# cmcqueen/lzs-compression

Measured on AMD Instinct MI355X. Metric: input GB/s on 64KiB blocks, bit-exact vs C ref, higher is better.
Workload: dtype u8

## Files before the change

lzs_compression_amd/csrc/kernels/compress_wg.inc:

```

#ifdef LZS_WGV_WG_WAVES
constexpr uint32_t kW = LZS_WGV_WG_WAVES;
#else
constexpr uint32_t kW = 4;
#endif
static_assert(kW == 4 || kW == 8, "four or eight waves per workgroup");
constexpr uint32_t kWgThreads  = 64u * kW;
constexpr uint32_t kChunkStride = 64u * kW;
constexpr uint32_t kWgRing      = kW == 8 ? 8192u : 4096u;
constexpr uint32_t kWgRingMask  = kWgRing - 1u, kWgRingWords = kWgRing / 4u;
constexpr uint32_t kRefillUnit  = 128u * kW;
#ifndef LZS_WG_HEAD3
#define LZS_WG_HEAD3 1792
#endif
#ifndef LZS_WG_HEAD2
#define LZS_WG_HEAD2 1024
#endif
#ifdef LZS_WGV_HEAD3
constexpr uint32_t kWgHead3    = LZS_WGV_HEAD3;
#else
constexpr uint32_t kWgHead3    = LZS_WG_HEAD3;
#endif
#ifdef LZS_WGV_HEAD2
constexpr uint32_t kWgHead2    = LZS_WGV_HEAD2;
#else
constexpr uint32_t kWgHead2    = LZS_WG_HEAD2;
#endif
#ifdef LZS_WGV_NO3
constexpr bool kNo3 = true;
#else
constexpr bool kNo3 = false;
#endif
#ifdef LZS_WGV_EXIT8
constexpr bool kExit8 = true;
typedef uint8_t exit_t;
#else
constexpr bool kExit8 = false;
typedef uint16_t exit_t;
#endif
#ifdef LZS_WGV_CHAIN_SAFE
constexpr bool kChainSafe = true;
#else
constexpr bool kChainSafe = false;
#endif
constexpr uint32_t kWgHead2Shift = kWgHead2 == 4096 ? 4 : kWgHead2 == 2048 ? 5 : kWgHead2 == 1024 ? 6 : kWgHead2 == 512 ? 7 : 8;
#ifdef LZS_WGV_POOL
constexpr uint32_t kWgPool     = LZS_WGV_POOL;
#else
constexpr uint32_t kWgPool     = 128u * kW;
#endif
static_assert(kWgPool == 128u * kW || (kW == 4 && kWgPool == 256), "a wave parses one or two chunks of 64 positions");
constexpr int      kCh         = (int)(kWgPool / kChunkStride);
constexpr uint32_t kWgLinkN    = (2047u + 2u * kWgPool + 63u) / 64u * 64u;
constexpr uint32_t kWgResN     = 2 * kWgPool;
constexpr uint32_t kWgBitWords = 64u * kW;
constexpr uint32_t kBitMask    = 32u * kWgBitWords - 1u;
constexpr uint32_t kOpen       = 0xFFFFu;
constexpr uint32_t kExtOpen    = 63;
#ifndef LZS_SUBSTEPS
#define LZS_SUBSTEPS 2
#endif
#ifdef LZS_WGV_SUBSTEPS
constexpr int kSubsteps = LZS_WGV_SUBSTEPS;
#else
constexpr int kSubsteps = LZS_SUBSTEPS;
#endif
#ifndef LZS_HOPS
#define LZS_HOPS 2
#endif
#ifdef LZS_WGV_HOPS
#define LZS_HOPS_HERE LZS_WGV_HOPS
#else
#define LZS_HOPS_HERE LZS_HOPS
#endif
constexpr int kHops = LZS_HOPS_HERE;
#ifdef LZS_WGV_HOP_END
constexpr bool kHopEnd = true;
#else
constexpr bool kHopEnd = false;
#endif
#ifdef LZS_WGV_HOPS_LAST
constexpr int kHopsLast = LZS_WGV_HOPS_LAST;
#else
constexpr int kHopsLast = kHops;
#endif
constexpr uint32_t kExtMax     = 59;
constexpr uint32_t kOpenStep   = 4080;
#ifndef LZS_RUN_ROUNDS
#define LZS_RUN_ROUNDS 2
#endif
#ifndef LZS_RUN_POOL
#define LZS_RUN_POOL 128
#endif
constexpr uint32_t kRunRounds  = LZS_RUN_ROUNDS;
constexpr uint32_t kRunPool    = LZS_RUN_POOL;

struct __attribute__((aligned(16))) BlkLds {
    uint32_t ring[kWgRingWords + 4];
    uint32_t head3[kNo3 ? 1 : kWgHead3];
    uint32_t head2[kWgHead2];
    uint16_t link3[kNo3 ? 2 : kWgLinkN];
    uint16_t link2[kWgLinkN];
    uint16_t res[kWgResN];
    exit_t   exitfn[kExit8 && kWgPool < 2u * kWgThreads ? 2u * kWgThreads : kWgPool];
    uint32_t bits[kWgBitWords];
    uint32_t chunk_bits[2 * kW];
    uint32_t nextp;
    uint32_t bcast[8];
#ifdef LZS_PAD_LDS
    uint32_t pad[LZS_PAD_LDS / 4];
#endif
};

#ifndef LZS_HASH3_MUL
#define LZS_HASH3_MUL 0x1EB419u
#endif
#ifndef LZS_HASH2_MUL
#define LZS_HASH2_MUL 0xCFC8AE9Bu
#endif
#ifdef LZS_WGV_HASH3_MUL
constexpr uint32_t kHash3Mul = LZS_WGV_HASH3_MUL;
#else
constexpr uint32_t kHash3Mul = LZS_HASH3_MUL;
#endif
#ifdef LZS_WGV_HASH2_MUL
constexpr uint32_t kHash2Mul = LZS_WGV_HASH2_MUL;
#else
constexpr uint32_t kHash2Mul = LZS_HASH2_MUL;
#endif
__device__ __forceinline__ uint32_t wg_hash3x4(uint32_t t) { return __umulhi(__umul24(t, kHash3Mul), 4u * kWgHead3) & ~3u; }

__device__ __forceinline__ uint32_t wg_slot_base(uint32_t B) { return ((B >> 6) % (kWgLinkN / 64u)) * 64u; }
__device__ __forceinline__ uint32_t wg_link_slot(uint32_t at)
{
    if constexpr ((kWgLinkN & (kWgLinkN - 1u)) == 0u) return at & (kWgLinkN - 1u);
    uint32_t b, r;
#ifdef LZS_WGV_LEAN
    asm("v_add_u16 %0, %2, %1" : "=v"(b) : "v"(at), "n"(kWgLinkN));
#else
    asm("v_add_u16 %0, %1, %2" : "=v"(b) : "v"(at), "v"(kWgLinkN));
#endif
    asm("v_min_u16 %0, %1, %2" : "=v"(r) : "v"(at), "v"(b));
    return r;
}

__device__ __forceinline__ uint32_t lcp12(uint32_t x0, uint32_t x1, uint32_t x2)
{
    uint32_t f0, f1, f2;
    asm("v_ffbl_b32 %0, %1" : "=v"(f0) : "v"(x0));
    asm("v_ffbl_b32 %0, %1" : "=v"(f1) : "v"(x1));
    asm("v_ffbl_b32 %0, %1" : "=v"(f2) : "v"(x2));
    const uint32_t a = f1 | 32u, b = f2 | 64u;
    const uint32_t m = f0 < a ? (f0 < b ? f0 : b) : (a < b ? a : b);
    return m >> 3;
}

__device__ __forceinline__ void bits_or(uint32_t *ring, uint32_t words, uint32_t at, uint32_t value, uint32_t width)
{
    const uint32_t sh = at & 31u, d = (at >> 5) & (words - 1);
    const uint64_t v = (uint64_t)value << (64u - sh - width);
    const uint32_t hi = (uint32_t)(v >> 32), lo = (uint32_t)v;
    __hip_atomic_fetch_or(&ring[d], hi, __ATOMIC_RELAXED, __HIP_MEMORY_SCOPE_WORKGROUP);
    if (lo) __hip_atomic_fetch_or(&ring[(d + 1) & (words - 1)], lo, __ATOMIC_RELAXED, __HIP_MEMORY_SCOPE_WORKGROUP);
}

struct WgOut {
    uint32_t flushed;
    uint32_t head;
    uint8_t *dst;
    uint32_t cap;
    bool     aligned4;
    uint32_t limit;
    bool     ored;
};

__device__ __forceinline__ uint32_t wg_bit_at(const WgOut &o) { return ((o.flushed << 3) + o.head) & kBitMask; }

__device__ __forceinline__ void wg_store_quarter(const WgOut &o, BlkLds &L, uint32_t lane)
{
    const uint32_t slot = ((o.flushed >> 8) & (kWgBitWords / 64u - 1u)) * 64u + lane;
    const uint32_t v = __builtin_bswap32(L.bits[slot]);
    L.bits[slot] = 0;
    const uint32_t at = o.flushed + 4 * lane;
    if (o.ored) {
        if (v) atomicOr(reinterpret_cast<unsigned int *>(o.dst + at), v);
        return;
    }
    if (o.aligned4 && at + 4 <= o.limit) {
        *reinterpret_cast<uint32_t *>(o.dst + at) = v;
    } else {
        for (uint32_t k = 0; k < 4; k++)
            if (at + k < o.limit) o.dst[at + k] = (uint8_t)(v >> (8 * k));
    }
}

__device__ __forceinline__ uint16_t *wg_dummy(BlkLds &L) { return reinterpret_cast<uint16_t *>(L.exitfn) + threadIdx.x; }

__device__ __forceinline__ uint32_t wg_ring_byte(const uint32_t *ring, uint32_t q) { return reinterpret_cast<const uint8_t *>(ring)[q & kWgRingMask]; }
__device__ __forceinline__ void wg_read12(const uint32_t *ring, uint32_t q, uint32_t &w0, uint32_t &w1, uint32_t &w2)
{
    const uint32_t a = (q & kWgRingMask) >> 2;
    const uint32_t d0 = ring[a], d1 = ring[a + 1], d2 = ring[a + 2], d3 = ring[a + 3];
    w0 = __builtin_amdgcn_alignbyte(d1, d0, q);
    w1 = __builtin_amdgcn_alignbyte(d2, d1, q);
    w2 = __builtin_amdgcn_alignbyte(d3, d2, q);
}

typedef __attribute__((address_space(3))) uint32_t lds_u32_t;
typedef __attribute__((address_space(3))) uint16_t lds_u16_t;
__device__ __forceinline__ uint32_t lds_off(const void *p) { return (uint32_t)(uintptr_t)(__attribute__((address_space(3))) const void *)p; }
__device__ __forceinline__ lds_u32_t *lds_word(uint32_t off) { return (lds_u32_t *)(uintptr_t)off; }
__device__ __forceinline__ lds_u16_t *lds_half(uint32_t off) { return (lds_u16_t *)(uintptr_t)off; }

__device__ __forceinline__ void wg_hash_range(BlkLds &L, uint32_t B0, uint32_t Be, uint32_t lane, uint32_t wave)
{
    const uint32_t head3_at = lds_off(L.head3), head2_at = lds_off(L.head2);
    const uint32_t dummy3 = lds_off(L.exitfn) + 4u * lane, dummy2 = dummy3 + 256u;
    for (uint32_t B = B0 + 64u * wave; B < Be; B += kChunkStride * kCh) {
        uint32_t e[kCh][5];
#pragma unroll
        for (int j = 0; j < kCh; j++) {
            const uint32_t p = B + kChunkStride * j + lane;
            const uint32_t a = ((p - 4u) & kWgRingMask) >> 2;
#pragma unroll
            for (int k = 0; k < 5; k++) e[j][k] = L.ring[a + k];
        }
#pragma unroll
        for (int j = 0; j < kCh; j++) {
            const uint32_t Bj = B + kChunkStride * j, p = Bj + lane;
            const uint32_t tcur = __builtin_amdgcn_alignbyte(e[j][2], e[j][1], p);
            const uint32_t rot = __builtin_amdgcn_alignbit(e[j][0], e[j][0], 8);
            const uint32_t x = (e[j][0] ^ rot) | (e[j][1] ^ e[j][0]) | (e[j][2] ^ e[j][0]) | (e[j][3] ^ e[j][0]) | (e[j][4] ^ e[j][0]);
            const bool skip = x == 0u;
            const uint32_t g2 = head2_at + (((tcur * kHash2Mul) >> (kWgHead2Shift - 2u)) & (4u * (kWgHead2 - 1)));
            const uint32_t a2 = skip ? dummy2 : g2;
            const uint32_t sl = wg_slot_base(Bj) + lane;
            uint16_t *const dummy16 = wg_dummy(L);
            if constexpr (!kNo3) {
                const uint32_t g3 = opaque(head3_at + wg_hash3x4(tcur));
                const uint32_t a3 = skip ? dummy3 : g3;
                *(Bj < Be ? &L.link3[sl] : dummy16) = (uint16_t)a3;
            }
            *(Bj < Be ? &L.link2[sl] : dummy16) = (uint16_t)a2;
        }
    }
}

template <int K>
__device__ __forceinline__ void wg_chain_group(BlkLds &L, uint32_t B, uint32_t &slot, uint32_t lane, uint32_t half, uint16_t *links)
{
    (void)half;
    uint32_t at[K], old[K];
    uint16_t *la[K];
#pragma unroll
    for (int j = 0; j < K; j++) {
        la[j] = &links[slot + lane];
        at[j] = *la[j];
        slot = slot + 64u >= kWgLinkN ? slot + 64u - kWgLinkN : slot + 64u;
    }
#pragma unroll
    for (int j = 0; j < K; j++) {
        const uint32_t p = B + 64u * j + lane;
        old[j] = __hip_atomic_exchange(lds_word(at[j]), p, __ATOMIC_RELAXED, __HIP_MEMORY_SCOPE_WORKGROUP);
    }
#pragma unroll
    for (int j = 0; j < K; j++) {
        const uint32_t p = B + 64u * j + lane;
        const uint32_t d = p - old[j] < kNoLink ? p - old[j] : kNoLink;
        *la[j] = (uint16_t)d;
    }
}

__device__ __forceinline__ void wg_chain_batch_safe(BlkLds &L, uint32_t B, uint32_t &slot, uint32_t lane, uint32_t half, uint16_t *links)
{
    (void)half;
    const uint32_t at = links[slot + lane];
    const uint32_t p = B + lane;
    const bool ins = at - lds_off(L.exitfn) >= (uint32_t)sizeof(L.exitfn);
    uint64_t same = __builtin_amdgcn_ballot_w64(ins);
#pragma unroll
    for (uint32_t bit = 2; bit < 15u; bit++) {
        const bool set = (at >> bit) & 1u;
        const uint64_t bb = __builtin_amdgcn_ballot_w64(set);
        same &= set ? bb : ~bb;
    }
    const uint64_t lower = same & ((1ull << lane) - 1ull);
    const bool top = (same >> lane >> 1) == 0ull;
    const uint32_t old = ins ? *lds_word(at) : ~0u;
    __builtin_amdgcn_wave_barrier();
    uint32_t d = kNoLink;
    if (ins) {
        if (lower) d = lane - (63u - (uint32_t)__builtin_clzll(lower));
        else       d = p - old < kNoLink ? p - old : kNoLink;
        if (top) *lds_word(at) = p;
    }
    links[slot + lane] = (uint16_t)d;
    slot = slot + 64u >= kWgLinkN ? slot + 64u - kWgLinkN : slot + 64u;
    __builtin_amdgcn_wave_barrier();
}

__device__ __forceinline__ void wg_chain_range(BlkLds &L, uint32_t B0, uint32_t Be, uint32_t lane, uint32_t wave)
{
    if (wave >= 2u) return;
    if (kNo3 && wave == 0u) return;
    const bool two = wave == 1u;
    uint16_t *const links = two ? L.link2 : L.link3;
    const uint32_t half = two ? 2u : 0u;
    uint32_t slot = wg_slot_base(B0);
    uint32_t B = B0;
    if constexpr (kChainSafe) {
        for (; B < Be; B += 64u) wg_chain_batch_safe(L, B, slot, lane, half, links);
        return;
    }
#ifdef LZS_WGV_PRIO
    __builtin_amdgcn_s_setprio(3);
#endif
    for (; B + 256u <= Be; B += 256u) wg_chain_group<4>(L, B, slot, lane, half, links);
    for (; B < Be; B += 64u) wg_chain_group<1>(L, B, slot, lane, half, links);
#ifdef LZS_WGV_PRIO
    __builtin_amdgcn_s_setprio(2);
#endif
}

#ifdef LZS_PROFILE
#ifdef LZS_PROFILE_COUNTS
#define SEARCH_PROF_PARAMS , uint32_t *prof_acc
#else
#define SEARCH_PROF_PARAMS , unsigned long long *prof_acc
#endif
#define SEARCH_PROF_ARGS , prof_acc
#else
#define SEARCH_PROF_PARAMS
#define SEARCH_PROF_ARGS
#endif
__device__ __forceinline__ void wg_extend(BlkLds &L, uint32_t Pb, uint32_t entry, uint32_t npos, uint32_t n, uint32_t lane, uint32_t wave,
                                          uint32_t (&rr)[2] SEARCH_PROF_PARAMS)
{
    PROF_ITER_DECL;
    constexpr uint32_t kRoom = kTokenMax + kExtMax + 1;
#pragma unroll
    for (int h = 0; h < kCh; h++) {
        const uint32_t gi = kChunkStride * h + 64u * wave + lane;
        rr[h] = 0;
        if (64u * wave + kChunkStride * h >= npos) continue;
        const uint32_t p = Pb + gi;
        const uint32_t k = L.res[p & (kWgResN - 1)];
        const uint32_t off = (0u - k) & 0xFFFu;
        const uint32_t len = off ? (k + 0xFFFu) >> 12 : 0u;
        const uint32_t r = off | (len << 11);
        const bool need = gi >= entry && gi < npos && len == kSearchCap && n - p > kSearchCap;
#ifdef LZS_ABLATE_EXTEND
        const uint64_t needs = 0ull;
#else
        const uint64_t needs = __builtin_amdgcn_ballot_w64(need);
#endif
        if (needs == 0ull) {
            rr[h] = r | ((len > kTokenMax ? len - kTokenMax : 0u) << 15);
            continue;
        }
        PROF_COUNT(19, 1);
        const uint32_t left = (uint32_t)__builtin_amdgcn_ds_bpermute((int)((lane - 1u) << 2), (int)r);
        const bool head = need && !(lane > 0u && ((needs >> (lane - 1u)) & 1ull) != 0ull && ((left ^ r) & 0x7FFFu) == 0u);
        const uint64_t heads_all = __builtin_amdgcn_ballot_w64(head);
        const uint64_t ends = (heads_all | ~needs) >> lane >> 1;
        const uint32_t runlen = ends ? (uint32_t)__builtin_ctzll(ends) : 63u - lane;
        uint32_t total = kSearchCap;
        if (head) {
            const uint32_t room = n - p < kRoom ? n - p : kRoom;
            total = kSearchCap + runlen < room ? kSearchCap + runlen : room;
            while (total < room) {
                PROF_ITER;
                uint32_t a0, a1, a2, b0, b1, b2;
                wg_read12(L.ring, p + total, a0, a1, a2);
                wg_read12(L.ring, p + total - off, b0, b1, b2);
                uint32_t e = lcp12(a0 ^ b0, a1 ^ b1, a2 ^ b2);
                e = e < 12u ? e : 12u;
                e = e < room - total ? e : room - total;
                total += e;
                if (e < 12u) break;
            }
        }
        PROF_ITER_DONE(27);
        const uint64_t heads = heads_all & ((2ull << lane) - 1ull);
        const uint32_t hp = heads ? 63u - (uint32_t)__builtin_clzll(heads) : lane;
        const uint32_t th = (uint32_t)__builtin_amdgcn_ds_bpermute((int)(hp << 2), (int)total);
        uint32_t ext = len >= kTokenMax ? len - kTokenMax : 0u;
        if (need) ext = th >= kRoom ? kExtOpen : th - (lane - hp) - kTokenMax;
        rr[h] = r | (ext << 15);
    }
}

struct Walk {
    uint32_t p, t0, t1, t2;
    uint32_t nreach, myslot;
    uint32_t nback;
    int32_t key;
    uint32_t cap;
    uint32_t nfirst2;
    const uint16_t *links;
    uint16_t *resp;
    uint32_t pb, probe;
};
constexpr int32_t kKeyNone3 = 0x2000, kKeyNone2 = 0x1000;

template <bool HE>
__device__ __forceinline__ void wg_search(BlkLds &L, Walk &W, uint32_t Pb, uint32_t pend, uint32_t n, uint32_t lane, bool lit, bool drain SEARCH_PROF_PARAMS)
{
    const uint32_t slot0 = wg_slot_base(Pb);
    uint16_t *const dummy = wg_dummy(L);
    PROF_ITER_DECL;
    bool pool_done = false;
    uint32_t p = W.p, t0 = W.t0, t1 = W.t1, t2 = W.t2, nreach = W.nreach, myslot = W.myslot;
    uint32_t nback = W.nback, cap = W.cap, nfirst2 = W.nfirst2;
    uint32_t pb = W.pb, probe = W.probe;
    int32_t key = W.key;
    const uint16_t *links = W.links;
    uint16_t *resp = W.resp;
#ifdef LZS_WGV_LEAN
    const uint32_t vFFF = 0xFFFu, vRC = kWgRingMask & ~3u, vRM = kWgRingMask;
#else
    const uint32_t vFFF = opaque(0xFFFu), vRC = opaque(kWgRingMask & ~3u);
    const uint32_t vRM = kWgRingMask == 0xFFFu ? vFFF : opaque(kWgRingMask);
#endif
    const uint8_t *const ring8 = reinterpret_cast<const uint8_t *>(L.ring);
    (void)vFFF; (void)vRM;
    for (;;) {
        const uint64_t idle = __builtin_amdgcn_ballot_w64(nback == 0u);
        const uint32_t nidle = (uint32_t)__builtin_popcountll(idle);
        if (!pool_done && nidle >= kRefillMin) {
            uint32_t basep = 0;
            if (lane == 0) asm volatile("ds_add_rtn_u32 %0, %1, %2\n\ts_waitcnt lgkmcnt(0)" : "=v"(basep) : "v"(lds_off(&L.nextp)), "v"(nidle) : "memory");
            basep = uniform(basep);
            pool_done = basep + nidle >= pend;
            const uint32_t rank = __builtin_amdgcn_mbcnt_hi((uint32_t)(idle >> 32),
                                  __builtin_amdgcn_mbcnt_lo((uint32_t)idle, 0u));
            const uint32_t np = basep + rank;
            const bool take = nback == 0u && np < pend;
            PROF_COUNT(9, 1);
            PROF_COUNT(10, __builtin_popcountll(__builtin_amdgcn_ballot_w64(take)));
            PROF_COUNT(43, __builtin_amdgcn_ballot_w64(take) == 0ull);
            PROF_T0;
            if (take) {
                *resp = (uint16_t)key;
                p = np;
                wg_read12(L.ring, p, t0, t1, t2);
                const uint32_t before = wg_ring_byte(L.ring, p - 1u);
                uint32_t sl = slot0 + (p - Pb);
                sl = sl >= kWgLinkN ? sl - kWgLinkN : sl;
                myslot = sl;
                const uint32_t l3 = kNo3 ? kNoLink : (uint32_t)L.link3[sl], l2 = L.link2[sl];
                const uint32_t lim = n - p < kSearchCap ? n - p : kSearchCap;
                const bool maybe1 = p >= 1u && ((t0 ^ ((t0 << 8) | before)) & 0xFFFFu) == 0;
                uint32_t len1 = 0;
                if (__builtin_amdgcn_ballot_w64(maybe1) != 0ull) {
                    PROF_ITER;
                    len1 = lcp12(t0 ^ ((t0 << 8) | before), t1 ^ ((t1 << 8) | (t0 >> 24)), t2 ^ ((t2 << 8) | (t1 >> 24)));
                    len1 = len1 < lim ? len1 : lim;
                }
                const bool seeded = maybe1 && len1 >= 2u;
                const bool capped = seeded && len1 == lim;
                const uint32_t reach = p < kWindow ? p : kWindow;
                nreach = ~reach;
#ifdef LZS_ABLATE_STEPS
                const bool walk3 = false, walk2 = false;
#else
                const bool walk3 = !kNo3 && lim >= 3u && !capped && l3 <= reach && (seeded || !lit);
                const bool walk2 = lim >= 2u && !capped && (kNo3 || !seeded) && l2 <= reach;
#endif
                nfirst2 = 0u - (walk2 ? l2 : kNoLink);
                nback = walk3 ? 0u - l3 : (walk2 ? nfirst2 : 0u);
                key = seeded ? (int32_t)((len1 << 12) - 1u) : (walk3 ? kKeyNone3 : kKeyNone2);
                cap = (walk3 || lit || kNo3) ? lim : 2u;
                links = walk3 ? L.link3 : L.link2;
                uint16_t *const slot = &L.res[p & (kWgResN - 1)];
                resp = slot;
                cap = (walk3 || walk2) ? cap : 0u;
#if LZS_HOPS_HERE
                pb = p + (((uint32_t)key + 0xFFFu) >> 12);
                probe = wg_ring_byte(L.ring, pb);
#endif
            }
            PROF_T1(14);
            PROF_ITER_DONE(18);
        }
        if (pool_done && __builtin_amdgcn_ballot_w64(nback != 0u && (drain || p < Pb)) == 0ull) break;
        PROF_COUNT(11, 1);
        PROF_COUNT(8 + 4, __builtin_popcountll(__builtin_amdgcn_ballot_w64(nback != 0u)));
        PROF_T0B;
#pragma unroll
        for (int sub = 0; sub < kSubsteps; sub++) {
#if LZS_HOPS_HERE
            const int nhops = (HE && sub == kSubsteps - 1) ? kHopsLast : kHops;
#pragma unroll
            for (int hop = 0; hop < nhops; hop++) {
                const uint32_t cb = ring8[(pb + nback) & vRM];
                const uint32_t ax = myslot + nback;
                const uint32_t nnx = nback - links[wg_link_slot(ax)];
                if constexpr (HE) {
                    const uint32_t nto = nnx > nreach ? nnx : 0u;
                    nback = cb != probe ? nto : nback;
                } else {
                    const bool skip = cb != probe && nnx > nreach;
                    nback = skip ? nnx : nback;
                }
            }
#endif
            uint32_t w0, w1, w2;
            {
                const uint32_t q = p + nback;
                const uint32_t *const wp = reinterpret_cast<const uint32_t *>(ring8 + (q & vRC));
                const uint32_t d0 = wp[0], d1 = wp[1], d2 = wp[2], d3 = wp[3];
                w0 = __builtin_amdgcn_alignbyte(d1, d0, q);
                w1 = __builtin_amdgcn_alignbyte(d2, d1, q);
                w2 = __builtin_amdgcn_alignbyte(d3, d2, q);
            }
            const uint32_t at = myslot + nback;
            const uint32_t nd = links[wg_link_slot(at)];
            uint32_t len = lcp12(w0 ^ t0, w1 ^ t1, w2 ^ t2);
            uint32_t capm = cap;
            if constexpr (HE) asm("v_min_u16 %0, %1, %2" : "=v"(capm) : "v"(cap), "v"(nback));
            asm("v_min_u16 %0, %1, %2" : "=v"(len) : "v"(len), "v"(capm));
            const int32_t cand = (int32_t)((len << 12) + nback);
            key = key > cand ? key : cand;
            const uint32_t nnext = nback - nd;
            const int32_t kend = opaque((len == capm || !(nnext > nreach)) ? key : 0);
            const bool fallback = !kNo3 && kend == kKeyNone3 && nfirst2 > nreach;
            const int32_t kfin = opaque(fallback ? 0 : kend);
            key = fallback ? kKeyNone2 : key;
            cap = fallback ? 2u : cap;
            links = fallback ? L.link2 : links;
            const uint32_t nwalk = fallback ? nfirst2 : nnext;
            if constexpr (!HE) {
                cap = kfin != 0 ? 0u : cap;
            }
            nback = kfin != 0 ? 0u : nwalk;
#if LZS_HOPS_HERE
            pb = p + (((uint32_t)key + vFFF) >> 12);
            probe = ring8[pb & vRM];
#endif
        }
        PROF_T1B(15);
    }
    *resp = (uint16_t)key;
    resp = nback == 0u ? dummy : resp;
    W.p = p; W.t0 = t0; W.t1 = t1; W.t2 = t2; W.nreach = nreach; W.myslot = myslot;
    W.nback = nback; W.key = key; W.cap = cap; W.nfirst2 = nfirst2;
    W.pb = pb; W.probe = probe;
    W.links = links; W.resp = resp;
}

struct WgJob {
    const uint8_t *src;
    uint32_t n, cend, c0, w0;
    bool last;
    uint32_t *out_len;
    uint32_t *exit_pos;
    unsigned long long *nbits;
    uint32_t *open_info;
#ifdef LZS_WGV_CHANNELS
    const uint8_t *hist;
    uint32_t hlen;
    uint8_t *status;
#endif
};

#ifdef LZS_WGV_CHANNELS
__device__ __forceinline__ uint32_t wg_view_byte(const WgJob &job, uint32_t q)
{
    return q < job.hlen ? job.hist[q] : (q < job.n ? job.src[q - job.hlen] : 0u);
}
__device__ __forceinline__ uint4 wg_view_load16(const WgJob &job, uint32_t p)
{
    const uint32_t h = job.hlen;
    if (p + 16u <= h) return load16(job.hist, p, h, ((uintptr_t)job.hist & 15u) == 0, ((uintptr_t)job.hist & 3u) == 0);
    if (p >= h) {
        if (p >= job.n) return make_uint4(0u, 0u, 0u, 0u);
        const uint8_t *q = job.src + (p - h);
        return load16(q, 0u, job.n - p, ((uintptr_t)q & 15u) == 0, ((uintptr_t)q & 3u) == 0);
    }
    uint32_t w[4] = {0u, 0u, 0u, 0u};
    for (uint32_t k = 0; k < 16u; k++) w[k >> 2] |= wg_view_byte(job, p + k) << (8u * (k & 3u));
    return make_uint4(w[0], w[1], w[2], w[3]);
}
__device__ __forceinline__ u32x4 wg_view_read16(const WgJob &job, uint32_t q)
{
    u32x4 v;
    if (q >= job.hlen) {
        __builtin_memcpy(&v, job.src + (q - job.hlen), 16);
    } else if (q + 16u <= job.hlen) {
        __builtin_memcpy(&v, job.hist + q, 16);
    } else {
        uint32_t w[4] = {0u, 0u, 0u, 0u};
        for (uint32_t k = 0; k < 16u; k++) w[k >> 2] |= wg_view_byte(job, q + k) << (8u * (k & 3u));
        v.x = w[0]; v.y = w[1]; v.z = w[2]; v.w = w[3];
    }
    return v;
}
#endif

template <int ENTRY = 0, bool HE = false>
__device__ __forceinline__ void wg_compress_job(BlkLds &L, const WgJob &job, WgOut o)
{
    const uint32_t tid  = threadIdx.x;
    const uint32_t lane = tid & 63u;
    const uint32_t wave = uniform(tid >> 6);
    const uint8_t *src = job.src;
    const uint32_t n   = job.n;
    const uint32_t cend = job.cend;
    const uint32_t head0 = o.head;
    const bool src16   = ((uintptr_t)src & 15u) == 0;
    const bool src4    = ((uintptr_t)src & 3u) == 0;
#ifdef LZS_WGV_CHANNELS
    (void)src16; (void)src4;
#endif

    for (uint32_t i = tid; i < (kNo3 ? 1u : kWgHead3); i += kWgThreads) L.head3[i] = ~0u;
    for (uint32_t i = tid; i < kWgHead2; i += kWgThreads) L.head2[i] = ~0u;
    L.bits[tid] = 0;
    if (tid == 0) L.ring[kWgRingWords - 1] = 0x00FF00FFu;
    __syncthreads();

    if (job.open_info && tid == 0) { job.open_info[0] = 0; job.open_info[1] = 0; }
    uint32_t c = job.c0;
    uint32_t loaded = job.w0;
    uint32_t next = job.w0;
#if !defined(LZS_NO_PREFETCH) && !defined(LZS_WGV_CHANNELS)
    const __amdgpu_buffer_rsrc_t src_rsrc = __builtin_amdgcn_make_buffer_rsrc((void *)src, 0, (int)n, 0x00020000);
    u32x4 pre = {0u, 0u, 0u, 0u};
    uint32_t pre_at = ~0u;
#endif
    PROF_DECL;

    Walk W;
    W.p = 0; W.t0 = W.t1 = W.t2 = 0; W.nreach = ~0u; W.myslot = 0;
    W.nback = 0; W.key = kKeyNone2; W.cap = 0; W.nfirst2 = 0u - kNoLink;
    W.pb = 0; W.probe = 0;
    W.links = L.link2; W.resp = wg_dummy(L);
    bool pending = false;
    uint32_t run_rounds = 0;
    bool lit_mode = false;
    uint32_t Pb = 0, pend = 0;
    const uint32_t nup = (cend + 63u) & ~63u;

    for (;;) {
        if (o.flushed >= o.cap) break;
        if (!pending && (c >= cend || next >= nup)) break;
        PROF_MARK(4);
        const bool fresh = next < nup;
        uint32_t Sb = next;
        if (!pending) while (Sb + 64 <= c) Sb += 64;
        const bool run_mode = !pending && run_rounds != 0u;
        const uint32_t pool = run_mode ? kRunPool : kWgPool;
        const uint32_t Se = fresh ? (Sb + pool < nup ? Sb + pool : nup) : Sb;
        if (fresh) {
            const uint32_t need = (Se > c ? Se : c) + 96;
            while (loaded < n && loaded < need) {
                PROF_COUNT(42, 1);
                if (wave == ((loaded / kRefillUnit) & (kW - 1u)) && lane < kRefillUnit / 16u) {
                    const uint32_t p = loaded + 16 * lane;
#if defined(LZS_WGV_CHANNELS)
                    const uint4 v = wg_view_load16(job, p);
#elif !defined(LZS_NO_PREFETCH)
                    const uint4 v = pre_at == loaded ? make_uint4(pre.x, pre.y, pre.z, pre.w) : load16(src, p, n, src16, src4);
#else
                    const uint4 v = load16(src, p, n, src16, src4);
#endif
                    const uint32_t at = (p & kWgRingMask) >> 2;
                    *reinterpret_cast<uint4 *>(&L.ring[at]) = v;
                    if (at == 0) *reinterpret_cast<uint4 *>(&L.ring[kWgRingWords]) = v;
                }
                loaded += kRefillUnit;
            }
#if !defined(LZS_NO_PREFETCH) && !defined(LZS_WGV_CHANNELS)
            if (src16 && loaded + kRefillUnit <= n) {
                pre = __builtin_amdgcn_raw_buffer_load_b128(src_rsrc, (int)(loaded + 16u * (lane & (kRefillUnit / 16u - 1u))), 0, 0);
                pre_at = loaded;
            }
#endif
            PROF_SYNC(32);
            PROF_MARK(0);
            { PROF_T0; PROF_COUNT(17, (Se - next) >> 6);
              for (uint32_t R = next; R < Se; R += kWgPool) {
                  const uint32_t R2 = R + kWgPool < Se ? R + kWgPool : Se;
                  if (R != next) PROF_SYNC(33);
#ifndef LZS_ABLATE_BUILD
                  wg_hash_range(L, R, R2, lane, wave);
                  PROF_SYNC(34);
                  wg_chain_range(L, R, R2, lane, (wave + blockIdx.x) & (kW - 1u));
#endif
              }
              PROF_T1(16); }
            next = Se;
        }
        const uint32_t send = Se < cend ? Se : cend;
        if (tid == 0) L.nextp = (!pending && c > Sb) ? c : Sb;
        PROF_SYNC(35);
        PROF_MARK(1);

#ifdef LZS_WGV_PRIO
        __builtin_amdgcn_s_setprio(0);
#endif
        wg_search<HE>(L, W, Sb, send, n, lane, lit_mode, run_mode && fresh SEARCH_PROF_ARGS);
#ifdef LZS_WGV_PRIO
        __builtin_amdgcn_s_setprio(2);
#endif
        PROF_MARK(2);
        PROF_SYNC(36);
        PROF_MARK(5);

        bool at_once = false;
        if (!pending) {
            Pb = Sb; pend = send; pending = fresh;
            if (!(run_mode && fresh)) continue;
            at_once = true;
            run_rounds--;
        }

#ifdef LZS_ABLATE_PARSE
        c = pend;
        Pb = Sb; pend = send; pending = fresh;
        continue;
#endif
        const uint32_t npos = pend - Pb;
        PROF_STAMP0;
        uint32_t rr[2];
        wg_extend(L, Pb, c - Pb, npos, n, lane, wave, rr SEARCH_PROF_ARGS);
        PROF_STAMP(20);
        while (c < pend && o.flushed < o.cap) {
            const uint32_t entry = c - Pb;
            PROF_COUNT(31, 1);
            uint32_t T4[2][6], t4[2], xc[2];
#pragma unroll
            for (int h = 0; h < kCh; h++) {
                const uint32_t cb = kChunkStride * h + 64u * wave;
                const uint32_t inside = cb < npos ? (npos - cb < 64u ? npos - cb : 64u) : 0u;
                const uint32_t r = rr[h];
                const uint32_t len = (r >> 11) & 15u, ext = r >> 15;
                uint32_t step = len < kTokenMax ? len : kTokenMax + ext;
                step = len < 2u ? 1u : step;
                const uint32_t land = lane + step;
                const uint32_t xb = kExit8 ? 0u : cb;
                uint32_t to = land < inside ? land : lane;
                uint32_t ex = xb + land;
                to = ext == kExtOpen ? lane : to;
                ex = ext == kExtOpen ? (kExit8 ? 192u + lane : (0x8000u | (cb + lane))) : ex;
                to = lane < inside ? to : lane;
                ex = lane < inside ? ex : xb + lane;
                t4[h] = to << 2;
                xc[h] = ex;
            }
#pragma unroll
            for (int d = 0; d < 6; d++) {
#pragma unroll
                for (int h = 0; h < kCh; h++) {
                    T4[h][d] = t4[h];
                    t4[h] = (uint32_t)__builtin_amdgcn_ds_bpermute((int)t4[h], (int)t4[h]);
                }
            }
#pragma unroll
            for (int h = 0; h < kCh; h++) {
                const uint32_t cb = kChunkStride * h + 64u * wave;
                L.exitfn[cb + lane] = (exit_t)__builtin_amdgcn_ds_bpermute((int)t4[h], (int)xc[h]);
            }
            PROF_STAMP(21);
            PROF_SYNC(37);
            PROF_STAMP(22);
            while (o.head >= 2048u) {
                PROF_COUNT(29, 1);
                if (wave == ((o.flushed >> 8) & (kW - 1u))) wg_store_quarter(o, L, lane);
                o.flushed += 256u;
                o.head -= 2048u;
            }
            uint32_t enter[2] = {0x100u, 0x100u};
            uint32_t last = entry;
            while (last < npos) {
                const uint32_t k = last >> 6;
                if (k == wave) enter[0] = last & 63u;
                if (kCh > 1 && k == wave + kW) enter[1] = last & 63u;
                PROF_COUNT(28, 1);
                const uint32_t v = uniform((uint32_t)L.exitfn[last]), from = last & ~63u;
                last = !kExit8 ? v : v < 192u ? from + v : (0x8000u | (from + v - 192u));
            }
            const uint32_t chain_end = (last & 0x8000u) ? kOpen : last;
            const uint32_t open_at = last & 0x7FFFu;
            PROF_STAMP(23);
            PROF_MARK(3);
            uint32_t n4[2];
            bool tok[2];
#pragma unroll
            for (int h = 0; h < kCh; h++) n4[h] = (enter[h] & 63u) << 2;
#pragma unroll
            for (int d = 0; d < 6; d++) {
                uint32_t via[2];
#pragma unroll
                for (int h = 0; h < kCh; h++)
                    via[h] = (uint32_t)__builtin_amdgcn_ds_bpermute((int)n4[h], (int)T4[h][d]);
#pragma unroll
                for (int h = 0; h < kCh; h++) n4[h] = ((lane >> d) & 1u) ? via[h] : n4[h];
            }
#pragma unroll
            for (int h = 0; h < kCh; h++) {
                const uint32_t before = (uint32_t)__builtin_amdgcn_update_dpp((int)~0u, (int)n4[h], 0x138, 0xf, 0xf, false);
                tok[h] = enter[h] < 64u && n4[h] != before;
            }
#if !defined(LZS_WGV_PACK_BY_CHUNK) && !(defined(LZS_WGV_POOL) && LZS_WGV_POOL == 256)
            const uint32_t nt0 = (uint32_t)__builtin_popcountll(__builtin_amdgcn_ballot_w64(tok[0]));
            const uint32_t nt1 = (uint32_t)__builtin_popcountll(__builtin_amdgcn_ballot_w64(tok[1]));
            uint32_t rec[2];
#pragma unroll
            for (int h = 0; h < 2; h++) rec[h] = (uint32_t)__builtin_amdgcn_ds_bpermute((int)n4[h], (int)rr[h]) | (n4[h] << 19);
            uint32_t valhi[2] = {0u, 0u}, vallo[2] = {0u, 0u}, width[2] = {0u, 0u}, incl[2] = {0u, 0u}, from1[2] = {0u, 0u};
            const uint32_t npass = nt0 + nt1 > 64u ? 2u : 1u;
            PROF_COUNT(30, npass - 1u);
#pragma unroll
            for (int ps = 0; ps < 2; ps++) {
                if ((uint32_t)ps >= npass) break;
                const uint32_t t = 64u * ps + lane;
                const uint32_t idx1 = t - nt0;
                const uint32_t pulled = (uint32_t)__builtin_amdgcn_ds_bpermute((int)((idx1 & 63u) << 2), (int)rec[1]);
                const bool f1 = t >= nt0;
                const bool valid = t < nt0 + nt1;
                const uint32_t rc = (ps == 0 && !f1) ? rec[0] : pulled;
                const uint32_t r = rc & 0x1FFFFFu, posc = rc >> 21;
                const uint32_t byte = wg_ring_byte(L.ring, Pb + (f1 ? kChunkStride : 0u) + 64u * wave + posc) & 0xFFu;
                const uint32_t len = (r >> 11) & 15u, ext = r >> 15, off = r & kWindow;
                const uint32_t ov = off <= kShortMax ? ((3u << 7) | off) : ((2u << 11) | off);
                const uint32_t ow = off <= kShortMax ? 9u : 13u;
                const uint32_t first = len < kTokenMax ? len : kTokenMax;
                const uint32_t lv = first <= 4u ? first - 2u : first + 7u;
                const uint32_t lw = first <= 4u ? 2u : 4u;
                const uint32_t full = (ext * 137u) >> 11;
                uint32_t tv = (((1u << (4u * full)) - 1u) << 4) | (ext - kNibbleMax * full);
                uint32_t tw = 4u * (full + 1u);
                tw = len < kTokenMax ? 0u : tw;
                tv = len < kTokenMax ? 0u : tv;
                uint32_t hv = (ov << lw) | lv, hw = ow + lw;
                hv = len < 2u ? byte : hv;
                hw = len < 2u ? 9u : hw;
                uint32_t w = hw + tw;
                w = ext == kExtOpen ? 0u : w;
                w = valid ? w : 0u;
                const uint64_t v = w ? (((uint64_t)hv << tw) | tv) : 0ull;
                valhi[ps] = (uint32_t)(v >> 32); vallo[ps] = (uint32_t)v; width[ps] = w; from1[ps] = f1 ? 1u : 0u;
                if (job.open_info) {
                    const uint32_t pos = Pb + (f1 ? kChunkStride : 0u) + 64u * wave + posc;
                    if (w && len >= kTokenMax && pos + kTokenMax + ext == n) { job.open_info[0] = off; job.open_info[1] = pos; }
                }
                incl[ps] = wave_inclusive_sum(w);
            }
            const uint32_t sum0 = (uint32_t)__builtin_amdgcn_readlane((int)incl[0], 63);
            const uint32_t bits0 = nt0 ? (uint32_t)__builtin_amdgcn_readlane((int)incl[0], (int)((nt0 - 1u) & 63u)) : 0u;
            const uint32_t sum_all = sum0 + (npass > 1u ? (uint32_t)__builtin_amdgcn_readlane((int)incl[1], 63) : 0u);
            if (lane == 63u) { L.chunk_bits[wave] = bits0; L.chunk_bits[kW + wave] = sum_all - bits0; }
            PROF_STAMP(24);
            PROF_SYNC(38);
            PROF_STAMP(25);
            const uint32_t cbits = lane < 2u * kW ? L.chunk_bits[lane & (2u * kW - 1u)] : 0u;
            const uint32_t cincl = wave_inclusive_sum(cbits);
            const uint32_t total = (uint32_t)__builtin_amdgcn_readlane((int)cincl, (int)(2u * kW - 1u));
            const uint32_t cexcl = cincl - cbits;
            const uint32_t at0 = wg_bit_at(o);
            const uint32_t before0 = (uint32_t)__builtin_amdgcn_readlane((int)cexcl, (int)wave);
            const uint32_t before1 = (uint32_t)__builtin_amdgcn_readlane((int)cexcl, (int)(kW + wave));
#pragma unroll
            for (int ps = 0; ps < 2; ps++) {
                if ((uint32_t)ps >= npass) break;
                const uint32_t carry = ps ? sum0 : 0u;
                const uint32_t rel = carry + incl[ps] - width[ps];
                const uint32_t at = (at0 + (from1[ps] ? before1 + rel - bits0 : before0 + rel)) & kBitMask;
                const uint64_t v = (((uint64_t)valhi[ps] << 32) | vallo[ps]) << ((64u - (at & 31u) - width[ps]) & 63u);
                const uint32_t vh = (uint32_t)(v >> 32), vl = (uint32_t)v;
                const uint32_t d = at >> 5;
                const uint32_t dh = vh ? d : tid, dl = vl ? (d + 1u) & (kWgBitWords - 1) : tid;
                __hip_atomic_fetch_or(&L.bits[dh], vh, __ATOMIC_RELAXED, __HIP_MEMORY_SCOPE_WORKGROUP);
                __hip_atomic_fetch_or(&L.bits[dl], vl, __ATOMIC_RELAXED, __HIP_MEMORY_SCOPE_WORKGROUP);
            }
#else
            uint32_t valhi[2], vallo[2], width[2], incl[2], rtok[2], btok[2];
#pragma unroll
            for (int h = 0; h < kCh; h++) {
                rtok[h] = (uint32_t)__builtin_amdgcn_ds_bpermute((int)n4[h], (int)rr[h]);
                btok[h] = wg_ring_byte(L.ring, Pb + kChunkStride * h + 64u * wave + (n4[h] >> 2)) & 0xFFu;
            }
#pragma unroll
            for (int h = 0; h < kCh; h++) {
                const uint32_t r = rtok[h];
                const uint32_t len = (r >> 11) & 15u, ext = r >> 15, off = r & kWindow;
                const uint32_t ov = off <= kShortMax ? ((3u << 7) | off) : ((2u << 11) | off);
                const uint32_t ow = off <= kShortMax ? 9u : 13u;
                const uint32_t first = len < kTokenMax ? len : kTokenMax;
                const uint32_t lv = first <= 4u ? first - 2u : first + 7u;
                const uint32_t lw = first <= 4u ? 2u : 4u;
                const uint32_t full = (ext * 137u) >> 11;
                uint32_t tv = (((1u << (4u * full)) - 1u) << 4) | (ext - kNibbleMax * full);
                uint32_t tw = 4u * (full + 1u);
                tw = len < kTokenMax ? 0u : tw;
                tv = len < kTokenMax ? 0u : tv;
                uint32_t hv = (ov << lw) | lv, hw = ow + lw;
                hv = len < 2u ? btok[h] : hv;
                hw = len < 2u ? 9u : hw;
                uint32_t w = hw + tw;
                w = ext == kExtOpen ? 0u : w;
                w = tok[h] ? w : 0u;
                const uint64_t v = w ? (((uint64_t)hv << tw) | tv) : 0ull;
                valhi[h] = (uint32_t)(v >> 32); vallo[h] = (uint32_t)v; width[h] = w;
                if (job.open_info) {
                    const uint32_t pos = Pb + kChunkStride * h + 64u * wave + (n4[h] >> 2);
                    if (w && len >= kTokenMax && pos + kTokenMax + ext == n) { job.open_info[0] = off; job.open_info[1] = pos; }
                }
                incl[h] = wave_inclusive_sum(w);
                if (lane == 63u) L.chunk_bits[kW * h + wave] = incl[h];
            }
            PROF_STAMP(24);
            PROF_SYNC(38);
            PROF_STAMP(25);
            const uint32_t cbits = lane < kW * kCh ? L.chunk_bits[lane & (2u * kW - 1u)] : 0u;
            const uint32_t cincl = wave_inclusive_sum(cbits);
            const uint32_t total = (uint32_t)__builtin_amdgcn_readlane((int)cincl, (int)(2u * kW - 1u));
            const uint32_t cexcl = cincl - cbits;
            const uint32_t at0 = wg_bit_at(o);
#pragma unroll
            for (int h = 0; h < kCh; h++) {
                const uint32_t before = (uint32_t)__builtin_amdgcn_readlane((int)cexcl, (int)(kW * h + wave));
                const uint32_t at = (at0 + before + incl[h] - width[h]) & kBitMask;
                const uint64_t v = (((uint64_t)valhi[h] << 32) | vallo[h]) << ((64u - (at & 31u) - width[h]) & 63u);
                const uint32_t vh = (uint32_t)(v >> 32), vl = (uint32_t)v;
                const uint32_t d = at >> 5;
                const uint32_t dh = vh ? d : tid, dl = vl ? (d + 1u) & (kWgBitWords - 1) : tid;
                __hip_atomic_fetch_or(&L.bits[dh], vh, __ATOMIC_RELAXED, __HIP_MEMORY_SCOPE_WORKGROUP);
                __hip_atomic_fetch_or(&L.bits[dl], vl, __ATOMIC_RELAXED, __HIP_MEMORY_SCOPE_WORKGROUP);
            }
#endif
            o.head += total;
#ifndef LZS_NO_LIT_MODE
            lit_mode = total > 8u * (npos - entry);
#endif
            PROF_STAMP(26);

            PROF_MARK(6);
            if (chain_end != kOpen) {
// ... 391 lines not shown
```

Baseline: 82.22.

## Interleave link3 and link2 chains into one paired LDS link array

Merges the separate link3 and link2 ring arrays into a single interleaved array so each position's two chain links sit in one 32-bit word. Slot setup then reads both links with one LDS load, and the walk tracks a byte offset ('mine') instead of a links pointer plus slot, so switching to the 2-byte chain is just setting an offset bit. This is meant to cut LDS reads and pointer registers in the hot match-walk loop. In exchange the chain-link stores become strided, and the wrap arithmetic now works in bytes with a 16-bit bound assertion.

```diff
diff --git a/lzs_compression_amd/csrc/kernels/compress_wg.inc b/lzs_compression_amd/csrc/kernels/compress_wg.inc
--- a/lzs_compression_amd/csrc/kernels/compress_wg.inc
+++ b/lzs_compression_amd/csrc/kernels/compress_wg.inc
@@ -52,6 +52,9 @@
 static_assert(kWgPool == 128u * kW || (kW == 4 && kWgPool == 256), "a wave parses one or two chunks of 64 positions");
 constexpr int      kCh         = (int)(kWgPool / kChunkStride);
 constexpr uint32_t kWgLinkN    = (2047u + 2u * kWgPool + 63u) / 64u * 64u;
+constexpr uint32_t kLinkHalves = kNo3 ? 1u : 2u, kLinkBytes = 2u * kLinkHalves, kLink2Half = kLinkHalves - 1u;
+constexpr uint32_t kLinkShift  = kNo3 ? 1u : 2u;
+constexpr uint32_t kLinkRingBytes = kLinkBytes * kWgLinkN;
 constexpr uint32_t kWgResN     = 2 * kWgPool;
 constexpr uint32_t kWgBitWords = 64u * kW;
 constexpr uint32_t kBitMask    = 32u * kWgBitWords - 1u;
@@ -99,8 +102,7 @@
     uint32_t ring[kWgRingWords + 4];
     uint32_t head3[kNo3 ? 1 : kWgHead3];
     uint32_t head2[kWgHead2];
-    uint16_t link3[kNo3 ? 2 : kWgLinkN];
-    uint16_t link2[kWgLinkN];
+    uint16_t link[kLinkHalves * kWgLinkN];
     uint16_t res[kWgResN];
     exit_t   exitfn[kExit8 && kWgPool < 2u * kWgThreads ? 2u * kWgThreads : kWgPool];
     uint32_t bits[kWgBitWords];
@@ -131,14 +133,15 @@
 __device__ __forceinline__ uint32_t wg_hash3x4(uint32_t t) { return __umulhi(__umul24(t, kHash3Mul), 4u * kWgHead3) & ~3u; }
 
 __device__ __forceinline__ uint32_t wg_slot_base(uint32_t B) { return ((B >> 6) % (kWgLinkN / 64u)) * 64u; }
-__device__ __forceinline__ uint32_t wg_link_slot(uint32_t at)
-{
-    if constexpr ((kWgLinkN & (kWgLinkN - 1u)) == 0u) return at & (kWgLinkN - 1u);
+__device__ __forceinline__ uint32_t wg_link_wrap(uint32_t at)
+{
+    if constexpr ((kWgLinkN & (kWgLinkN - 1u)) == 0u) return at & (kLinkRingBytes - 1u);
+    static_assert(2u * kLinkRingBytes <= 0x8000u, "the wrap is 16-bit arithmetic");
     uint32_t b, r;
 #ifdef LZS_WGV_LEAN
-    asm("v_add_u16 %0, %2, %1" : "=v"(b) : "v"(at), "n"(kWgLinkN));
-#else
-    asm("v_add_u16 %0, %1, %2" : "=v"(b) : "v"(at), "v"(kWgLinkN));
+    asm("v_add_u16 %0, %2, %1" : "=v"(b) : "v"(at), "n"(kLinkRingBytes));
+#else
+    asm("v_add_u16 %0, %1, %2" : "=v"(b) : "v"(at), "v"(kLinkRingBytes));
 #endif
     asm("v_min_u16 %0, %1, %2" : "=v"(r) : "v"(at), "v"(b));
     return r;
@@ -211,6 +214,7 @@
 __device__ __forceinline__ uint32_t lds_off(const void *p) { return (uint32_t)(uintptr_t)(__attribute__((address_space(3))) const void *)p; }
 __device__ __forceinline__ lds_u32_t *lds_word(uint32_t off) { return (lds_u32_t *)(uintptr_t)off; }
 __device__ __forceinline__ lds_u16_t *lds_half(uint32_t off) { return (lds_u16_t *)(uintptr_t)off; }
+__device__ __forceinline__ uint32_t wg_link_read(const BlkLds &L, uint32_t at) { return *lds_half(lds_off(L.link) + at); }
 
 __device__ __forceinline__ void wg_hash_range(BlkLds &L, uint32_t B0, uint32_t Be, uint32_t lane, uint32_t wave)
 {
@@ -234,14 +238,14 @@
             const bool skip = x == 0u;
             const uint32_t g2 = head2_at + (((tcur * kHash2Mul) >> (kWgHead2Shift - 2u)) & (4u * (kWgHead2 - 1)));
             const uint32_t a2 = skip ? dummy2 : g2;
-            const uint32_t sl = wg_slot_base(Bj) + lane;
+            uint16_t *const entry = &L.link[kLinkHalves * (wg_slot_base(Bj) + lane)];
             uint16_t *const dummy16 = wg_dummy(L);
             if constexpr (!kNo3) {
                 const uint32_t g3 = opaque(head3_at + wg_hash3x4(tcur));
                 const uint32_t a3 = skip ? dummy3 : g3;
-                *(Bj < Be ? &L.link3[sl] : dummy16) = (uint16_t)a3;
-            }
-            *(Bj < Be ? &L.link2[sl] : dummy16) = (uint16_t)a2;
+                *(Bj < Be ? entry : dummy16) = (uint16_t)a3;
+            }
+            *(Bj < Be ? entry + kLink2Half : dummy16) = (uint16_t)a2;
         }
     }
 }
@@ -254,7 +258,7 @@
     uint16_t *la[K];
 #pragma unroll
     for (int j = 0; j < K; j++) {
-        la[j] = &links[slot + lane];
+        la[j] = &links[kLinkHalves * (slot + lane)];
         at[j] = *la[j];
         slot = slot + 64u >= kWgLinkN ? slot + 64u - kWgLinkN : slot + 64u;
     }
@@ -274,7 +278,7 @@
 __device__ __forceinline__ void wg_chain_batch_safe(BlkLds &L, uint32_t B, uint32_t &slot, uint32_t lane, uint32_t half, uint16_t *links)
 {
     (void)half;
-    const uint32_t at = links[slot + lane];
+    const uint32_t at = links[kLinkHalves * (slot + lane)];
     const uint32_t p = B + lane;
     const bool ins = at - lds_off(L.exitfn) >= (uint32_t)sizeof(L.exitfn);
     uint64_t same = __builtin_amdgcn_ballot_w64(ins);
@@ -294,7 +298,7 @@
         else       d = p - old < kNoLink ? p - old : kNoLink;
         if (top) *lds_word(at) = p;
     }
-    links[slot + lane] = (uint16_t)d;
+    links[kLinkHalves * (slot + lane)] = (uint16_t)d;
     slot = slot + 64u >= kWgLinkN ? slot + 64u - kWgLinkN : slot + 64u;
     __builtin_amdgcn_wave_barrier();
 }
@@ -304,7 +308,7 @@
     if (wave >= 2u) return;
     if (kNo3 && wave == 0u) return;
     const bool two = wave == 1u;
-    uint16_t *const links = two ? L.link2 : L.link3;
+    uint16_t *const links = L.link + (two ? kLink2Half : 0u);
     const uint32_t half = two ? 2u : 0u;
     uint32_t slot = wg_slot_base(B0);
     uint32_t B = B0;
@@ -392,12 +396,11 @@
 
 struct Walk {
     uint32_t p, t0, t1, t2;
-    uint32_t nreach, myslot;
+    uint32_t nreach, mine;
     uint32_t nback;
     int32_t key;
     uint32_t cap;
     uint32_t nfirst2;
-    const uint16_t *links;
     uint16_t *resp;
     uint32_t pb, probe;
 };
@@ -410,11 +413,10 @@
     uint16_t *const dummy = wg_dummy(L);
     PROF_ITER_DECL;
     bool pool_done = false;
-    uint32_t p = W.p, t0 = W.t0, t1 = W.t1, t2 = W.t2, nreach = W.nreach, myslot = W.myslot;
+    uint32_t p = W.p, t0 = W.t0, t1 = W.t1, t2 = W.t2, nreach = W.nreach, mine = W.mine;
     uint32_t nback = W.nback, cap = W.cap, nfirst2 = W.nfirst2;
     uint32_t pb = W.pb, probe = W.probe;
     int32_t key = W.key;
-    const uint16_t *links = W.links;
     uint16_t *resp = W.resp;
 #ifdef LZS_WGV_LEAN
     const uint32_t vFFF = 0xFFFu, vRC = kWgRingMask & ~3u, vRM = kWgRingMask;
@@ -447,8 +449,14 @@
                 const uint32_t before = wg_ring_byte(L.ring, p - 1u);
                 uint32_t sl = slot0 + (p - Pb);
                 sl = sl >= kWgLinkN ? sl - kWgLinkN : sl;
-                myslot = sl;
-                const uint32_t l3 = kNo3 ? kNoLink : (uint32_t)L.link3[sl], l2 = L.link2[sl];
+                uint32_t l3 = kNoLink, l2;
+                if constexpr (kNo3) {
+                    l2 = L.link[sl];
+                } else {
+                    const uint32_t pair = reinterpret_cast<const uint32_t *>(L.link)[sl];
+                    l3 = pair & 0xFFFFu;
+                    l2 = pair >> 16;
+                }
                 const uint32_t lim = n - p < kSearchCap ? n - p : kSearchCap;
                 const bool maybe1 = p >= 1u && ((t0 ^ ((t0 << 8) | before)) & 0xFFFFu) == 0;
                 uint32_t len1 = 0;
@@ -471,7 +479,7 @@
                 nback = walk3 ? 0u - l3 : (walk2 ? nfirst2 : 0u);
                 key = seeded ? (int32_t)((len1 << 12) - 1u) : (walk3 ? kKeyNone3 : kKeyNone2);
                 cap = (walk3 || lit || kNo3) ? lim : 2u;
-                links = walk3 ? L.link3 : L.link2;
+                mine = kLinkBytes * sl + (walk3 ? 0u : 2u * kLink2Half);
                 uint16_t *const slot = &L.res[p & (kWgResN - 1)];
                 resp = slot;
                 cap = (walk3 || walk2) ? cap : 0u;
@@ -494,8 +502,8 @@
 #pragma unroll
             for (int hop = 0; hop < nhops; hop++) {
                 const uint32_t cb = ring8[(pb + nback) & vRM];
-                const uint32_t ax = myslot + nback;
-                const uint32_t nnx = nback - links[wg_link_slot(ax)];
+                const uint32_t ax = mine + (nback << kLinkShift);
+                const uint32_t nnx = nback - wg_link_read(L, wg_link_wrap(ax));
                 if constexpr (HE) {
                     const uint32_t nto = nnx > nreach ? nnx : 0u;
                     nback = cb != probe ? nto : nback;
@@ -514,8 +522,8 @@
                 w1 = __builtin_amdgcn_alignbyte(d2, d1, q);
                 w2 = __builtin_amdgcn_alignbyte(d3, d2, q);
             }
-            const uint32_t at = myslot + nback;
-            const uint32_t nd = links[wg_link_slot(at)];
+            const uint32_t at = mine + (nback << kLinkShift);
+            const uint32_t nd = wg_link_read(L, wg_link_wrap(at));
             uint32_t len = lcp12(w0 ^ t0, w1 ^ t1, w2 ^ t2);
             uint32_t capm = cap;
             if constexpr (HE) asm("v_min_u16 %0, %1, %2" : "=v"(capm) : "v"(cap), "v"(nback));
@@ -528,7 +536,7 @@
             const int32_t kfin = opaque(fallback ? 0 : kend);
             key = fallback ? kKeyNone2 : key;
             cap = fallback ? 2u : cap;
-            links = fallback ? L.link2 : links;
+            if constexpr (!kNo3) mine = fallback ? mine | 2u : mine;
             const uint32_t nwalk = fallback ? nfirst2 : nnext;
             if constexpr (!HE) {
                 cap = kfin != 0 ? 0u : cap;
@@ -543,10 +551,10 @@
     }
     *resp = (uint16_t)key;
     resp = nback == 0u ? dummy : resp;
-    W.p = p; W.t0 = t0; W.t1 = t1; W.t2 = t2; W.nreach = nreach; W.myslot = myslot;
+    W.p = p; W.t0 = t0; W.t1 = t1; W.t2 = t2; W.nreach = nreach; W.mine = mine;
     W.nback = nback; W.key = key; W.cap = cap; W.nfirst2 = nfirst2;
     W.pb = pb; W.probe = probe;
-    W.links = links; W.resp = resp;
+    W.resp = resp;
 }
 
 struct WgJob {
@@ -632,10 +640,10 @@
     PROF_DECL;
 
     Walk W;
-    W.p = 0; W.t0 = W.t1 = W.t2 = 0; W.nreach = ~0u; W.myslot = 0;
+    W.p = 0; W.t0 = W.t1 = W.t2 = 0; W.nreach = ~0u; W.mine = 2u * kLink2Half;
     W.nback = 0; W.key = kKeyNone2; W.cap = 0; W.nfirst2 = 0u - kNoLink;
     W.pb = 0; W.probe = 0;
-    W.links = L.link2; W.resp = wg_dummy(L);
+    W.resp = wg_dummy(L);
     bool pending = false;
     uint32_t run_rounds = 0;
     bool lit_mode = false;
```

Result: no change. 82.62, median of 6 (+0.5%).
